# Abhipray/audio-codec

Measured on AMD Instinct MI355X. Metric: audio channel-frames/s encode (48 kHz, 1024-line long blocks, 128 kb/s/ch), higher is better.
Workload: dtype f64

## Files before the change

### audio-codec_amd/csrc/k_psy.hip

```cpp
#include "pacx_launch.h"
#include "mdct_dev.h"
#include "pcm_stage.h"
#include "wave_np_sum.h"
#include "quant_dev.h"


template <int DT>
__device__ __forceinline__ double hann_sample(const typename PcmStage<DT>::elem *raw, int i,
                                              const double *__restrict__ hw,
                                              const double *__restrict__ hw_pcm)
{
    if constexpr (DT == 0) {
        const int c = raw[i];
        return hw_pcm[i] * (double)(c == -32768 ? 0 : c);
    } else {
        return hw[i] * raw[i];
    }
}

#ifdef PACX_PSY_DEBUG
__device__ long long g_psy_dbg[16 * 16];
#define PSY_T(k) do { long long t_; asm volatile("s_waitcnt lgkmcnt(0)\n\ts_memtime %0\n\ts_waitcnt lgkmcnt(0)" : "=s"(t_) :: "memory"); \
                      if (dbg_on) dbg_acc[k] += t_ - dbg_last; dbg_last = t_; } while (0)
extern "C" int pacx_debug_read_psy(long long *out, int n)
// ... 4 lines not shown
                       if (lane == 0 && side_last) atomicAdd((unsigned long long *)&g_psy_dbg[128 + (k)], (unsigned long long)(t_ - side_last)); \
                       side_last = t_; } while (0)
#else
#define PSY_T(k) do { } while (0)
#define SIDE_T(k) do { } while (0)
#endif

#ifdef MASK_NOINLINE_RT
__device__ __attribute__((noinline)) double mask_round_trip(double x) { return pacx_spl_of_intensity_of(x); }
#else
__device__ __forceinline__ double mask_round_trip(double x) { return pacx_spl_of_intensity_of(x); }
#endif

__device__ __forceinline__ PacxPeak make_peak(double left, double centre, int f, double fstep)
{
    const double e = left + centre;
    const double spl = pacx_spl_scalar(e);
    const double avg = (((double)(f - 1) * fstep) * left + ((double)f * fstep) * centre) / e;
    PacxPeak p;
    p.z = pacx_bark(avg);
    p.spl = spl;
    p.slope = -27.0 + 0.367 * fmax(spl - 40.0, 0.0);
    return p;
}

template <int DT> struct SideLongLds {
    typedef typename PcmStage<DT>::elem E;
    static constexpr int RAW_BYTES = (int)sizeof(E) * PACX_N_LONG;
    static constexpr int A_BYTES = 1024;
    static constexpr int B_BYTES = RAW_BYTES > 1032 * 8 ? RAW_BYTES : 1032 * 8;
    static constexpr int BYTES = A_BYTES + B_BYTES;
};

__device__ __forceinline__ void fft512n_g2(cplx a[8], cplx b[8], cplx *tile, const cplx tw1[7], const cplx tw2[7],
                                           int lane)
{
    dft8(a);
    dft8(b);
#pragma unroll
    for (int k1 = 1; k1 < 8; ++k1) {
        const cplx w = tw1[k1 - 1];
        a[k1] = c_mul(a[k1], w);
        b[k1] = c_mul(b[k1], w);
    }
    fft512n_x1_write(tile, a, lane);
    wave_lds_fence();
    fft512n_x1_read(tile, a, lane);
    fft512n_x1_write(tile, b, lane);
    dft8(a);
    wave_lds_fence();
    fft512n_x1_read(tile, b, lane);
    dft8(b);
#pragma unroll
    for (int k2 = 1; k2 < 8; ++k2) {
        const cplx w = tw2[k2 - 1];
        a[k2] = c_mul(a[k2], w);
        b[k2] = c_mul(b[k2], w);
    }
    fft512n_x2_write(tile, a, lane);
    wave_lds_fence();
    fft512n_x2_read(tile, a, lane);
    fft512n_x2_write(tile, b, lane);
    dft8(a);
    wave_lds_fence();
    fft512n_x2_read(tile, b, lane);
    wave_lds_fence();
    dft8(b);
}

__device__ __forceinline__ double bperm_f64(double v, int src_lane)
{
    const int lo = __builtin_amdgcn_ds_bpermute(src_lane << 2, __double2loint(v));
    const int hi = __builtin_amdgcn_ds_bpermute(src_lane << 2, __double2hiint(v));
    return __hiloint2double(hi, lo);
}

__device__ __forceinline__ double pair_intensity(cplx a, cplx bz, cplx w, double norm)
{
    const cplx s = make_double2(a.x + bz.x, a.y - bz.y);
    const cplx d = make_double2(a.x - bz.x, a.y + bz.y);
    const cplx wd = c_mul(w, d);
    const double xr = 0.5 * (s.x + wd.y), xi = 0.5 * (s.y - wd.x);
    return norm * fma(xr, xr, xi * xi);
}

__device__ __forceinline__ void load_lane_twiddles(const PacxTables &T, int lane, cplx tw1[7], cplx tw2[7])
{
#pragma unroll
    for (int k = 1; k < 8; ++k) {
        tw1[k - 1] = T.w512[(lane * k) & 511];
        tw2[k - 1] = T.w512[(8 * (lane & 7) * k) & 511];
    }
}

struct FrontArgs {
    const short *src;
    double *lines;
    int32_t *scale_out;
    uint32_t *status;
};
struct MdctOperands {
    int q[16];
    double w[16];
    cplx twl[8];
};

__device__ __forceinline__ void mdct_fetch(const PacxTables &T, const short *__restrict__ src, int lane,
                                           MdctOperands &m)
{
    const double *__restrict__ win = T.win_long;
#pragma unroll
    for (int j = 0; j < 4; ++j) {
        const int4 t = *(const int4 *)(src + 8 * (lane + 64 * j));
        m.q[4 * j] = t.x; m.q[4 * j + 1] = t.y; m.q[4 * j + 2] = t.z; m.q[4 * j + 3] = t.w;
    }
#pragma unroll
    for (int n1 = 0; n1 < 8; ++n1) {
        int i0, i1, i2, i3, ia, ib;
        mdct_fold_index<PACX_N_LONG>(n1, lane + 64 * n1, i0, i1, i2, i3);
        mdct_fold_sym_index(n1, i0, i1, i2, i3, ia, ib);
        m.w[2 * n1] = win[ia];
        m.w[2 * n1 + 1] = win[ib];
    }
#pragma unroll
    for (int k = 0; k < 8; ++k)
        m.twl[k] = T.tw_long[lane + 64 * k];
}

__device__ __forceinline__ void mdct_long_one(const PacxTables &T, long long cf, char *regB, int lane,
                                              const MdctOperands &m, double *__restrict__ lines,
                                              int32_t *__restrict__ scale_out, uint32_t *__restrict__ status)
{
    short *raw = (short *)regB;
    cplx *tile = (cplx *)regB;
    cplx tw1[7], tw2[7];
#pragma unroll
    for (int k = 1; k < 8; ++k)
        tw1[k - 1] = T.w512[(lane * k) & 511];
#pragma unroll
    for (int j = 0; j < 4; ++j)
        *(int4 *)(raw + 8 * (lane + 64 * j)) = make_int4(m.q[4 * j], m.q[4 * j + 1], m.q[4 * j + 2], m.q[4 * j + 3]);
    wave_lds_fence();
    cplx v[8];
    for (int pass = 0;; ++pass) {
        int lowest = 0;
#pragma unroll
        for (int n1 = 0; n1 < 8; ++n1) {
            int i0, i1, i2, i3;
            mdct_fold_index<PACX_N_LONG>(n1, lane + 64 * n1, i0, i1, i2, i3);
            double c0, c1, c2, c3;
            mdct_fold_codes<false>(raw, i0, i1, i2, i3, c0, c1, c2, c3, lowest);
            const double wa = m.w[2 * n1] * MDCT_LONG_KSCALE, wb = m.w[2 * n1 + 1] * MDCT_LONG_KSCALE;
            v[n1] = c_mul(mdct_fold_sym(n1, wa, wb, c0, c1, c2, c3), m.twl[n1]);
        }
        if (pass || !__builtin_amdgcn_ballot_w64(lowest == -32768))
            break;
        wave_lds_fence();
        mdct_zero_min_codes((unsigned *)raw, lane);
        wave_lds_fence();
    }
#pragma unroll
    for (int k = 1; k < 8; ++k)
        tw2[k - 1] = T.w512[(8 * (lane & 7) * k) & 511];
    wave_lds_fence();
    fft512n(v, tile, tw1, 1, tw2, 1, lane);
    mdct_long_epilogue(T, v, [&](int k3) { return m.twl[k3]; }, cf, lane, lines, scale_out, PACX_SUB, status);
}

template <int DT, bool FAST, bool FRONT = false>
__device__ __forceinline__ void side_long_one(const PacxTables &T, const PacxPcmView &in, long long cf,
                                              char *regA, char *regB, int lane,
                                              PacxPeak *__restrict__ peaks, int32_t *__restrict__ n_peaks,
                                              int32_t *__restrict__ n_kept_out,
                                              double *__restrict__ sbr_mean,
                                              int32_t *__restrict__ sbr_overall,
                                              const FrontArgs *fa = nullptr)
{
    typedef typename PcmStage<DT>::elem E;
    cplx *tile = (cplx *)regB;
    double *inten = (double *)regB;
    E *raw = (E *)regB;

#ifdef PACX_PSY_DEBUG
    long long side_last = 0;
#endif
    SIDE_T(15);
    const double *__restrict__ hw = T.hann_long, *__restrict__ hwp = T.hann_long_pcm;
    cplx ev[8], od[8];
    cplx tw1[7], tw2[7];
    load_lane_twiddles(T, lane, tw1, tw2);
    if constexpr (DT == 0 && FAST) {
        const long long f = cf / in.n_ch;
        const int ch = (int)(cf - f * in.n_ch);
        const short *src = (const short *)in.base + f * in.frame_stride + ch * in.ch_stride;
        int2 q[8];
#pragma unroll
        for (int n1 = 0; n1 < 8; ++n1)
            q[n1] = *(const int2 *)(src + 4 * (lane + 64 * n1));
        SIDE_T(0);
#pragma unroll
        for (int n1 = 0; n1 < 8; ++n1) {
            const int i = 4 * (lane + 64 * n1);
            const double2 h01 = *(const double2 *)(hwp + i), h23 = *(const double2 *)(hwp + i + 2);
            const int c0 = (short)(q[n1].x & 0xFFFF), c1 = q[n1].x >> 16;
            const int c2 = (short)(q[n1].y & 0xFFFF), c3 = q[n1].y >> 16;
            ev[n1] = make_double2(h01.x * (double)(c0 == -32768 ? 0 : c0), h01.y * (double)(c1 == -32768 ? 0 : c1));
            od[n1] = make_double2(h23.x * (double)(c2 == -32768 ? 0 : c2), h23.y * (double)(c3 == -32768 ? 0 : c3));
        }
    } else {
        stage_samples<DT, FAST>(raw, in, cf, 0, PACX_N_LONG, lane);
        wave_lds_fence();
        SIDE_T(0);
#pragma unroll
        for (int n1 = 0; n1 < 8; ++n1) {
            const int i = 4 * (lane + 64 * n1);
            ev[n1] = make_double2(hann_sample<DT>(raw, i, hw, hwp), hann_sample<DT>(raw, i + 1, hw, hwp));
            od[n1] = make_double2(hann_sample<DT>(raw, i + 2, hw, hwp), hann_sample<DT>(raw, i + 3, hw, hwp));
        }
        wave_lds_fence();
    }
    SIDE_T(1);
    fft512n_g2(ev, od, tile, tw1, tw2, lane);
    SIDE_T(2);
    const int mirror = (64 - lane) & 63;
    constexpr int AHEAD = 2;
    cplx w1q[8], w2q[8];
#pragma unroll
    for (int k3 = 0; k3 < AHEAD; ++k3) {
        w1q[k3] = T.w1024[lane + 64 * k3];
        w2q[k3] = T.w2048[lane + 64 * k3];
    }
#pragma unroll
    for (int k3 = 0; k3 < 8; ++k3) {
        const int k = lane + 64 * k3;
        if (k3 + AHEAD < 8) {
            w1q[k3 + AHEAD] = T.w1024[k + 64 * AHEAD];
            w2q[k3 + AHEAD] = T.w2048[k + 64 * AHEAD];
        }
        const cplx w1k = w1q[k3], w2k = w2q[k3];
        const cplx t = c_mul(w1k, od[k3]);
        const cplx zk = c_add(ev[k3], t), zk5 = c_sub(ev[k3], t);
        cplx pe, po;
        pe.x = bperm_f64(ev[7 - k3].x, mirror);
        pe.y = bperm_f64(ev[7 - k3].y, mirror);
        po.x = bperm_f64(od[7 - k3].x, mirror);
        po.y = bperm_f64(od[7 - k3].y, mirror);
        if (lane == 0) {
            pe = ev[(8 - k3) & 7];
            po = od[(8 - k3) & 7];
        }
        const cplx tm = c_mul(make_double2(-w1k.x, w1k.y), po);
        cplx zm = c_add(pe, tm), zm5 = c_sub(pe, tm);
        if (k == 0) {
            zm5 = zk;
            zm = zk5;
// ... 148 lines not shown
            const double mean = wave_np_sum(inten + T.band_lower_long[b], cnt, lane) / (double)cnt;
            if (lane == 0)
                sbr_mean[cf * PACX_SUB + (b - first)] = mean;
        }
        if (lane == 0) {
            const int sf = pacx_scale_factor(sqrt(mx / T.norm_long) / (double)PACX_M_LONG, T.n_scale_bits, 5);
            if (sf < sbr_overall[cf * PACX_SUB])
                sbr_overall[cf * PACX_SUB] = sf;
        }
    }
}

template <int DT, bool FAST>
__global__ __launch_bounds__(64, DT == 0 ? 3 : 2) void k_side_long(PacxTables T, PacxPcmView in,
                                                 const uint8_t *__restrict__ flags, long long n_cf,
                                                 int skip_cur, PacxPeak *__restrict__ peaks,
                                                 int32_t *__restrict__ n_peaks,
                                                 int32_t *__restrict__ n_kept_out,
                                                 double *__restrict__ sbr_mean,
                                                 int32_t *__restrict__ sbr_overall)
{
    __shared__ __attribute__((aligned(16))) char regA[SideLongLds<DT>::A_BYTES];
    __shared__ __attribute__((aligned(16))) char regB[SideLongLds<DT>::B_BYTES];
    const long long cf = pacx_xcd_frame(blockIdx.x, gridDim.x, n_cf);
    if (cf >= n_cf)
        return;
    const unsigned fl = flags ? flags[cf / in.n_ch] : 0u;
    if (skip_cur && (fl & 2u))
        return;
    side_long_one<DT, FAST>(T, in, cf, regA, regB, threadIdx.x, peaks, n_peaks, n_kept_out, sbr_mean,
                            sbr_overall);
}

__global__ __launch_bounds__(64, 3) void k_front_long(PacxTables T, PacxPcmView in, long long n_cf,
                                                      double *__restrict__ lines, int32_t *__restrict__ scale_out,
                                                      uint32_t *__restrict__ status, PacxPeak *__restrict__ peaks,
                                                      int32_t *__restrict__ n_peaks, int32_t *__restrict__ n_kept_out)
{
    __shared__ __attribute__((aligned(16))) char regA[SideLongLds<0>::A_BYTES];
    __shared__ __attribute__((aligned(16))) char regB[SideLongLds<0>::B_BYTES];
    static_assert(SideLongLds<0>::B_BYTES >= (int)sizeof(cplx) * WFFT_TILE_N, "region B holds the FFT tile");
    const long long cf = pacx_xcd_frame(blockIdx.x, gridDim.x, n_cf);
    if (cf >= n_cf)
        return;
    const int lane = threadIdx.x;
    if (lane == 0)
        status[cf] = 0u;
    if (lane >= 1 && lane < PACX_SUB)
        scale_out[cf * PACX_SUB + lane] = 0;
    const long long f = cf / in.n_ch;
    const int ch = (int)(cf - f * in.n_ch);
    FrontArgs fa;
    fa.src = (const short *)in.base + f * in.frame_stride + ch * in.ch_stride;
    fa.lines = lines;
    fa.scale_out = scale_out;
    fa.status = status;
    side_long_one<0, true, true>(T, in, cf, regA, regB, lane, peaks, n_peaks, n_kept_out, nullptr, nullptr,
                                 &fa);
}

template <int DT, bool FAST>
__global__ __launch_bounds__(64) void k_side_short(PacxTables T, PacxPcmView in,
                                                  const uint8_t *__restrict__ flags, long long n_cf,
                                                  int only_cur, PacxPeak *__restrict__ peaks,
                                                  int32_t *__restrict__ n_peaks,
                                                  int32_t *__restrict__ n_kept_out)
{
// ... 710 lines not shown
```

### audio-codec_amd/_lib.py

```python
import ctypes
import os

HERE = os.path.dirname(os.path.abspath(__file__))
LIB_PATH = os.environ.get("PACX_LIB") or os.path.join(HERE, "libpacx.so")

PACX_ABI_VERSION = 7
PCM_I16, PCM_F64 = 0, 1
FLAG_LAST, FLAG_CUR, FLAG_NEXT = 1, 2, 4
ST_SHORT, ST_ZERO_SUBBLOCK, ST_ALLOC_CAP, ST_VQ_UNDEFINED, ST_GUARD, ST_MALFORMED = 1, 2, 4, 8, 16, 32
ST_REF_RAISES = 64
ST_RATE_CAP = 128
RATE_STEP = 32
RATE_TARGET_GRID = 64
BAND_CAND = 16
PROFILE_MAX = 8193
SEG_CF_MAX = 1 << 40
E_ARG, E_UNSUPPORTED = -1, -2
REF_SCALAR_SBR_ERROR = "'numpy.int64' object does not support item assignment"
MAX_BANDS = 32
SUB = 8

c_double_p = ctypes.POINTER(ctypes.c_double)
c_int32_p = ctypes.POINTER(ctypes.c_int32)

# ... 144 lines not shown
    "profile_segments": [_I64, _I64, _D, _D, _P, _P],
    "pick": [_D, _P, _P, _P, _P],
    "pick_segments": [_I64, _I64, _P, _P, _P, _P, _P],
    "thresholds": [_D, _D, _P, _P, _P, _P],
    "pick_thresholds": [_D, _D, _D, _P, _P, _P, _P],
    "pick_thresholds_segments": [_I64, _I64, _D, _D, _P, _P, _P, _P, _P],
}
SIGNATURES.update({f"pacx_{kind}_{op}": (ctypes.c_int, [_P, _I64, *head, _P, _P, _P, *tail])
                   for kind, head in CURVE_HEADS.items() for op, tail in CURVE_TAILS.items()})


class PacxBucket(ctypes.Structure):
    _fields_ = [("drain_q16", ctypes.c_int64), ("size_bytes", ctypes.c_int64), ("start_q16", ctypes.c_int64)]


BUCKET_Q = 16
BUCKET_SIZE_MAX = 1 << 40
BUCKET_RESULT = ("total", "peak_q16", "peak_hop", "first_over", "end_q16")
BUCKET_SIGNATURES = {"pacx_bucket_scan": (ctypes.c_int, [_P, _I64, ctypes.c_int32, _P, ctypes.POINTER(PacxBucket), _P, _P,
                                                         _P])}
BUCKET_SIGNATURES.update({f"pacx_{kind}_solve_bucket": (ctypes.c_int, [_P, _I64, ctypes.c_int32, *head, _P, _P, _P, _I64,
                                                                       ctypes.POINTER(PacxBucket), _D, _D, _P, _P, _P, _P,
                                                                       _P, _P])
                          for kind, head in CURVE_HEADS.items()})
PIN_PHASES_MAX = 16
PIN_RESULT = ("phases", "open")
BUCKET_PIN_SIGNATURES = {"pacx_bucket_through": (ctypes.c_int, [_P, _I64, ctypes.c_int32, _P, ctypes.POINTER(PacxBucket), _P,
                                                                _P, _P, _P])}
BUCKET_PIN_SIGNATURES.update({f"pacx_{kind}_solve_bucket_pinned": (ctypes.c_int, [_P, _I64, ctypes.c_int32, *head, _P, _P, _P,
                                                                                  _I64, ctypes.POINTER(PacxBucket), _D, _D,
                                                                                  ctypes.c_int32, ctypes.c_int32, _P, _P,
                                                                                  _P, _P, _P, _P, _P, _P, _P])
                              for kind, head in CURVE_HEADS.items()})
NMR_MAX_BANDS, NMR_COUNT, NMR_AUDIBLE, NMR_MAX, NMR_HIST, NMR_HIST_BINS = 32, 0, 1, 2, 3, 320
NMR_HIST_LO, NMR_HIST_STEP = -120.0, 0.5
NMR_SUMMARY_WORDS = NMR_HIST + NMR_HIST_BINS + 2
INDEX_SEGMENT = 8192
(WIN_SINE, WIN_START, WIN_STOP, WIN_STARTSTOP, WIN_SINE_SHORT, WIN_HANN, WIN_HANN_SHORT, WIN_KBD,
 WIN_KBD_SHORT) = range(9)
MDCT_SHORT, MDCT_PREWINDOWED, MDCT_KBD = 1, 2, 4

_lib = None


class PacxError(RuntimeError):
    pass


def load():
    global _lib
    if _lib is not None:
        return _lib
    from . import build as _build
    if os.environ.get("PACX_LIB"):
        if _build._read(LIB_PATH + ".hash") != _build.library_hash():
            raise PacxError(f"{LIB_PATH} (PACX_LIB) was not built from the sources in this tree: rebuild it with "
                            "`python audio-codec_amd/build.py --variant ...` / `--phase-debug`")
    elif not _build.is_current():
        if os.environ.get("PACX_AUTOBUILD") == "1":
            import sys
            print("audio_codec_amd: libpacx.so is missing or stale -- rebuilding (PACX_AUTOBUILD=1)", file=sys.stderr,
                  flush=True)
            try:
                _build.build(verbose=False)
            except Exception as e:
                raise PacxError(f"libpacx.so is missing or stale and could not be rebuilt: {e}") from e
        else:
            raise PacxError("libpacx.so is missing or does not belong to the sources in this tree (content hash "
                            "mismatch): run `python audio-codec_amd/build.py` (or set PACX_AUTOBUILD=1).  "
                            "There is no CPU implementation of this path.")
    if not os.path.exists(LIB_PATH):
        raise PacxError(
            f"{LIB_PATH} not found: build it with `python audio-codec_amd/build.py` "
            "(hipcc, gfx950).  There is no CPU implementation of this path.")
    import torch
    lib = ctypes.CDLL(LIB_PATH)
    for name, (res, args) in {**SIGNATURES, **BUCKET_SIGNATURES, **BUCKET_PIN_SIGNATURES}.items():
        fn = getattr(lib, name)
        fn.restype = res
        fn.argtypes = args
    if lib.pacx_abi_version() != PACX_ABI_VERSION:
        raise PacxError("libpacx.so ABI version does not match the Python binding")
    _lib = lib
    return lib


def check(lib, handle, rc, what):
    if rc != 0:
        msg = lib.pacx_last_error(handle)
        raise PacxError(f"{what} failed ({rc}): {msg.decode() if msg else '?'}")
```

### audio-codec_amd/build.py

```python
import fcntl
import hashlib
import json
import os
import re
import subprocess
import sys
from concurrent.futures import ThreadPoolExecutor

HERE = os.path.dirname(os.path.abspath(__file__))
CSRC = os.path.join(HERE, "csrc")
OUT = os.path.join(HERE, "libpacx.so")
OBJ = os.path.join(HERE, "build")
RESOURCES = os.path.join(OBJ, "resources.json")
SOURCES = ["pacx_api.hip", "k_mdct.hip", "k_psy.hip", "k_quant.hip", "k_misc.hip", "k_mdct2.hip", "k_decode.hip",
           "k_vq.hip", "k_vq_dec.hip", "k_mdct3.hip", "k_index.hip", "k_nmr.hip", "k_rate.hip", "k_band.hip",
           "k_vq_band.hip", "k_profile.hip", "k_seg_profile.hip", "k_rate_profile.hip", "k_kept.hip",
           "k_bucket.hip", "k_bucket_pin.hip"]
FLAGS = ["-O3", "-std=c++17", "--offload-arch=gfx950", "-fPIC", "-ffp-contract=off",
         "-Wall", "-Wno-unused-function", "-Rpass-analysis=kernel-resource-usage"]


def _hipcc():
    return os.environ.get("HIPCC", "/opt/rocm/bin/hipcc")


def _headers():
    hs = sorted(os.path.join(CSRC, f) for f in os.listdir(CSRC) if f.endswith(".h"))
    hs += [os.path.join(HERE, "..", "include", f) for f in ("pacx.h", "pacx_bucket.h", "pacx_bucket_pin.h")]
    return hs


def _digest(paths, extra=()):
    h = hashlib.sha256()
    for e in extra:
        h.update(e.encode() + b"\0")
    for p in paths:
        h.update(os.path.basename(p).encode() + b"\0")
        with open(p, "rb") as f:
            h.update(f.read())
    return h.hexdigest()


def _read(path):
    try:
        with open(path) as f:
            return f.read().strip()
    except OSError:
        return None


def source_hashes(extra_flags=()):
    hs = _headers()
    return {s: _digest([os.path.join(CSRC, s)] + hs, FLAGS + list(extra_flags)) for s in SOURCES}


def library_hash():
    sh = source_hashes()
    return hashlib.sha256("".join(sh[s] for s in SOURCES).encode()).hexdigest()


def is_current():
# ... 189 lines not shown
```

### audio-codec_amd/csrc/k_misc.hip

```cpp
#include "pacx_launch.h"

__global__ void k_window(const double *__restrict__ win, long long n_rows, int len,
                         const double *__restrict__ x, double *__restrict__ y)
{
    const long long i = (long long)blockIdx.x * blockDim.x + threadIdx.x;
    if (i < n_rows * len)
        y[i] = win[i % len] * x[i];
}

__global__ void k_quant_elem(int op, long long n, const double *__restrict__ x, int scale, int a, int b,
                             int64_t *__restrict__ out)
{
    const long long i = (long long)blockIdx.x * blockDim.x + threadIdx.x;
    if (i >= n)
        return;
    const double v = x[i];
    if (op == 0) {
        const int64_t mag = pacx_quant_mag(fabs(v), a);
        out[i] = (v < 0.0 ? ((int64_t)1 << (a - 1)) : 0) + mag;
    } else if (op == 1) {
        out[i] = pacx_scale_factor(fabs(v), a, b);
    } else if (op == 2) {
        out[i] = pacx_mantissa(v, scale, a, b);
    } else {
        out[i] = pacx_mantissa_fp(v, scale, a, b);
    }
}

__global__ void k_dequant_elem(int op, long long n, const int64_t *__restrict__ codes, int scale, int a, int b,
                               double *__restrict__ out)
{
    const long long i = (long long)blockIdx.x * blockDim.x + threadIdx.x;
    if (i >= n)
// ... 290 lines not shown
    if (lane == 63) {
        ws[wv] = ss;
        wl[wv] = sl;
    }
    __syncthreads();
    int at_s = ss - ns, at_l = sl - nl, all_s = 0, all_l = 0;
#pragma unroll
    for (int w = 0; w < NW; ++w) {
        at_s += w < wv ? ws[w] : 0;
        at_l += w < wv ? wl[w] : 0;
        all_s += ws[w];
        all_l += wl[w];
    }
    for (int j = 0; j < per; ++j) {
        if (!((valid >> j) & 1ull))
            break;
        const long long f = f0 + j;
        if ((shorts >> j) & 1ull) {
            for (int c = 0; c < n_ch; ++c)
                list_short[at_s * n_ch + c] = (int32_t)(f * n_ch + c);
            ++at_s;
        } else {
            for (int c = 0; c < n_ch; ++c)
                list_long[at_l * n_ch + c] = (int32_t)(f * n_ch + c);
            ++at_l;
        }
    }
    if (tid == 0) {
        counts[0] = all_l * n_ch;
        counts[1] = all_s * n_ch;
    }
}

void pacx_k::pacx_launch_frame_lists(const uint8_t *flags, long long n_frames, int n_ch, int32_t *list_long,
                             int32_t *list_short, int32_t *counts, hipStream_t st)
{
    if (n_frames <= 0)
        return;
    if (n_frames <= LISTS_SMALL_MAX) {
        hipLaunchKernelGGL(k_frame_lists_small, dim3(1), dim3(LISTS_SMALL_THREADS), 0, st, flags, n_frames, n_ch, list_long,
                           list_short, counts);
        return;
    }
    (void)hipMemsetAsync(counts, 0, 2 * sizeof(int32_t), st);
    hipLaunchKernelGGL(k_frame_lists, dim3((unsigned)((n_frames + 255) / 256)), dim3(256), 0, st, flags, n_frames,
                       n_ch, list_long, list_short, counts);
}

void pacx_k::pacx_launch_transient_f64(long long n_blocks, int n_ch, int n, const double *blocks, double thresh, uint8_t *out,
                               hipStream_t st)
{
    if (n_blocks > 0)
        hipLaunchKernelGGL(k_transient_f64, dim3((unsigned)n_blocks), dim3(64), 0, st, n_blocks, n_ch, n, blocks, thresh,
                           out);
}

void pacx_k::pacx_launch_transient(const PacxPcmView &in, long long n_hops, int hop, uint8_t *transient,
                           uint8_t *flags, hipStream_t st)
{
    if (n_hops > 0)
        hipLaunchKernelGGL(k_transient, dim3((unsigned)n_hops), dim3(64), 0, st, in, n_hops, hop, transient);
    if (flags)
        hipLaunchKernelGGL(k_stream_flags, dim3((unsigned)((n_hops + 2 + 255) / 256)), dim3(256), 0, st,
                           transient, n_hops, flags);
}

// ... 40 lines not shown
```

### audio-codec_amd/csrc/pacx_api.hip

```cpp
#include <hip/hip_runtime.h>

#include <math.h>
#include <stdio.h>
#include <stdlib.h>
#include <string.h>

#include <cmath>
#include <string>
#include <vector>

#include "../../include/pacx.h"
#include "body_index.h"
#include "pacx_launch.h"
#include "pvq_dev.h"
#include "pacx_vq_tables.h"
#include "pacx_tables_gen.h"

using namespace pacx_k;

struct PacxOverrides {
    int split_short;
    int fuse_tail;
    int fuse_front;
    int vq_fuse_alloc;
    int vq_frame;
    int vq_bfs;
    int vq_dec_frame;
};

#define PACX_FUSE_FRONT_DEFAULT 1

static int env_override(const char *name, int lo, int hi)
{
    const char *e = getenv(name);
    if (!e || !*e)
        return -1;
    char *end;
    const long v = strtol(e, &end, 10);
    return (*end || v < lo || v > hi) ? -1 : (int)v;
}

static PacxOverrides read_overrides(void)
{
    PacxOverrides o;
    o.split_short = env_override("PACX_SPLIT_SHORT", 0, 0);
// ... 229 lines not shown
    int n_dev = 0;
    if (hipGetDeviceCount(&n_dev) != hipSuccess || n_dev <= 0)
        return fail(nullptr, PACX_E_HIP, "pacx_create: no HIP device visible (this library has no CPU path)");
    if (cfg->device < 0 || cfg->device >= n_dev)
        return fail(nullptr, PACX_E_ARG, "pacx_create: device ordinal out of range");

    pacx_handle *h = new pacx_handle();
    h->device = cfg->device;
    h->force = read_overrides();
    h->tables_exact = 1;
    memset(&h->T, 0, sizeof(h->T));
    int rc = PACX_OK;
#define TRY(x) do { rc = (x); if (rc) { g_create_err = h->err; pacx_destroy(h); return rc; } } while (0)
    {
        hipError_t e = hipSetDevice(cfg->device);
        if (e != hipSuccess) {
            g_create_err = std::string("hipSetDevice: ") + hipGetErrorString(e);
            delete h;
            return PACX_E_HIP;
        }
    }
    if (hipStreamCreateWithFlags(&h->side_stream, hipStreamNonBlocking) != hipSuccess ||
        hipEventCreateWithFlags(&h->ev_fork, hipEventDisableTiming) != hipSuccess ||
        hipEventCreateWithFlags(&h->ev_join, hipEventDisableTiming) != hipSuccess ||
        hipStreamCreateWithFlags(&h->short_stream, hipStreamNonBlocking) != hipSuccess ||
        hipStreamCreateWithFlags(&h->spare_stream, hipStreamNonBlocking) != hipSuccess ||
        hipEventCreateWithFlags(&h->ev_short_done, hipEventDisableTiming) != hipSuccess ||
        hipEventCreateWithFlags(&h->ev_lists, hipEventDisableTiming) != hipSuccess) {
        g_create_err = "pacx_create: could not create the side stream / events";
        pacx_destroy(h);
        return PACX_E_HIP;
    }
    {
        hipDeviceProp_t prop;
        h->n_cu = (hipGetDeviceProperties(&prop, cfg->device) == hipSuccess && prop.multiProcessorCount > 0)
                      ? prop.multiProcessorCount : 256;
    }
    PacxTables &T = h->T;
    const int NL = PACX_N_LONG, NS = PACX_N_SHORT, ML = PACX_M_LONG, MS = PACX_M_SHORT;
    const double sr = cfg->sample_rate;

    std::vector<double> wl(4 * NL), ws(NS), hl(NL), hs(NS);
    if (cfg->win_long) {
        memcpy(wl.data(), cfg->win_long, sizeof(double) * 4 * NL);
    } else {
        const std::vector<double> sl = gen_table(PACX_GEN_SINE_LONG, NL), ss = gen_table(PACX_GEN_SINE_SHORT, NS);
        const int pad = NL / 4 - NS / 4;
        for (int i = 0; i < NL; ++i) {
            wl[i] = sl[i];
            double st;
            if (i < NL / 2) st = sl[i];
            else if (i < NL / 2 + pad) st = 1.0;
            else if (i < NL / 2 + pad + NS / 2) st = ss[NS / 2 + (i - NL / 2 - pad)];
            else st = 0.0;
            wl[NL + i] = st;
            double ssw;
            if (i < pad) ssw = 0.0;
            else if (i < pad + NS / 2) ssw = ss[i - pad];
            else if (i < pad + NS / 2 + 2 * pad) ssw = 1.0;
            else if (i < pad + NS + 2 * pad) ssw = ss[NS / 2 + (i - pad - NS / 2 - 2 * pad)];
            else ssw = 0.0;
            wl[3 * NL + i] = ssw;
        }
        for (int i = 0; i < NL; ++i)
            wl[2 * NL + i] = wl[NL + (NL - 1 - i)];
    }
// ... 757 lines not shown
        return post_launch_forked(h, what);
    }
    if (!mixed && fast && (h->force.fuse_front >= 0 ? h->force.fuse_front : PACX_FUSE_FRONT_DEFAULT)) {
        s.front_long(st);
        s.mask(0, fuse ? &mt : nullptr, st);
        if (!fuse)
            tail(s.list_short, s.counts + 1, fuse, st);
        return post_launch(h, what);
    }
    const bool one_stream = !h->fork_side;
    hipStream_t side_st = one_stream ? st : h->side_stream;
    if (!one_stream) {
        HIP_TRY_FORKED(h, hipEventRecord(h->ev_fork, st));
        HIP_TRY_FORKED(h, hipStreamWaitEvent(h->side_stream, h->ev_fork, 0));
    }
    s.side(0, false, side_st);
    if (!one_stream)
        HIP_TRY_FORKED(h, hipEventRecord(h->ev_join, h->side_stream));
    s.mdct(st);
    if (!one_stream)
        HIP_TRY_FORKED(h, hipStreamWaitEvent(st, h->ev_join, 0));
    s.mask(0, fuse ? &mt : nullptr, st);
    if (!fuse || mixed)
        tail(s.list_short, s.counts + 1, fuse, st);
    return post_launch_forked(h, what);
}

extern "C" int pacx_set_side_fork(pacx_handle *h, int enable)
{
    if (!h)
        return PACX_E_ARG;
    h->fork_side = enable ? 1 : 0;
    return PACX_OK;
}

extern "C" int pacx_encode_batch(pacx_handle *h, const pacx_pcm *in, const uint8_t *frame_flags,
                                 int32_t *overall_scale, int32_t *scale_factor, int32_t *bit_alloc,
                                 int32_t *mantissa, uint32_t *status, void *stream)
{
    return encode_scalar(h, in, frame_flags, overall_scale, scale_factor, bit_alloc, mantissa, status, nullptr,
                         nullptr, stream, "pacx_encode_batch");
}

extern "C" int pacx_encode_pack_batch(pacx_handle *h, const pacx_pcm *in, const uint8_t *frame_flags,
                                      int32_t *overall_scale, int32_t *scale_factor, int32_t *bit_alloc,
                                      int32_t *mantissa, uint32_t *status, uint8_t *payload, int32_t *n_bytes,
                                      void *stream)
{
    if (h && in && in->n_frames > 0 && (!payload || !n_bytes))
        return fail(h, PACX_E_ARG, "pacx_encode_pack_batch: payload and n_bytes are required");
    return encode_scalar(h, in, frame_flags, overall_scale, scale_factor, bit_alloc, mantissa, status, payload,
                         n_bytes, stream, "pacx_encode_pack_batch");
}

extern "C" int pacx_encode_vq_batch(pacx_handle *h, const pacx_pcm *in, const uint8_t *frame_flags,
                                    int32_t *overall_scale, int32_t *bit_alloc, uint8_t *payload,
                                    int32_t *n_bytes, uint32_t *status, pacx_vq_entry *entries,
                                    int32_t *entry_count, int32_t entries_per_band, void *stream)
{
    if (!h)
        return PACX_E_ARG;
    EncodeStep s(h, frame_flags, stream);
    int rc = s.view(in);
    if (rc || s.n_cf == 0)
        return rc;
    if (!overall_scale || !bit_alloc || !payload || !n_bytes || !status)
// ... 1492 lines not shown
```

### audio-codec_amd/csrc/pacx_launch.h

```cpp
#ifndef PACX_LAUNCH_H
#define PACX_LAUNCH_H

#include "../../include/pacx.h"
#include "pacx_dev.h"

struct PvqTables;

namespace pacx_k {

void pacx_launch_mdct(const PacxTables &T, const PacxPcmView &in, int dtype, int fast,
                      const uint8_t *flags, long long n_cf, int short_blocks, int mixed, int prewin,
                      double *lines, int32_t *scale_out, int scale_stride, uint32_t *status,
                      hipStream_t st);
void pacx_launch_mdct_v2(const PacxTables &T, const PacxPcmView &in, const uint8_t *flags, long long n_cf,
                         int skip_cur, double *lines, int32_t *scale_out, int scale_stride,
                         uint32_t *status_init, int n_cu, const int32_t *cf_list, const int32_t *cf_count,
                         hipStream_t st);
void pacx_launch_mdct_x2(const PacxTables &T, const PacxPcmView &in, long long n_cf, double *lines,
                         int32_t *scale_out, int scale_stride, uint32_t *status_init, int n_cu, hipStream_t st);

void pacx_launch_side(const PacxTables &T, const PacxPcmView &in, int dtype, int fast,
                      const uint8_t *flags, long long n_cf, int short_blocks, int mixed,
                      PacxPeak *peaks, int32_t *n_peaks, int32_t *n_kept, double *sbr_mean,
                      int32_t *sbr_overall, hipStream_t st);
// ... 17 lines not shown
                          uint32_t *status, hipStream_t st);
void pacx_launch_quantize(const PacxTables &T, const uint8_t *flags, int n_ch, long long n_cf,
                          int short_blocks, int mixed, const double *lines, const int32_t *overall,
                          int overall_stride, const int32_t *bit_alloc, int32_t *scale_factor,
                          int32_t *mantissa, hipStream_t st);
void pacx_launch_pack(const PacxTables &T, const uint8_t *flags, int n_ch, long long n_cf,
                      const int32_t *overall, const int32_t *scale_factor, const int32_t *bit_alloc,
                      const int32_t *mantissa, const uint32_t *status, uint8_t *payload,
                      int payload_stride, int32_t *n_bytes, hipStream_t st);
void pacx_launch_tail(const PacxTables &T, const uint8_t *flags, int n_ch, long long n_cf, const double *smr,
                      const double *lines, const int32_t *overall, int32_t *bit_alloc, int32_t *scale_factor,
                      int32_t *mantissa, uint32_t *status, uint8_t *payload, int payload_stride,
                      int32_t *n_bytes, const int32_t *list_short, const int32_t *count_short, int skip_long,
                      hipStream_t st);
void pacx_launch_gather(long long n_cf, const uint8_t *payload, int payload_stride,
                        const int32_t *n_bytes, long long *chunk_buf, long long *offs_buf, uint8_t *body,
                        long long capacity, long long *total, hipStream_t st);

void pacx_launch_frame_lists(const uint8_t *flags, long long n_frames, int n_ch, int32_t *list_long,
                             int32_t *list_short, int32_t *counts, hipStream_t st);
void pacx_launch_window(const double *win, long long n_rows, int len, const double *x, double *y,
                        hipStream_t st);
void pacx_launch_quant_elem(int op, long long n, const double *x, int scale, int a, int b, int64_t *out,
                            hipStream_t st);
void pacx_launch_dequant_elem(int op, long long n, const int64_t *codes, int scale, int a, int b, double *out,
                              hipStream_t st);
void pacx_launch_mdct_direct(long long n_rows, int a, int b, int inverse, const double *x, double *y, hipStream_t st);
void pacx_launch_bitalloc_generic(long long n, int nb, const int32_t *n_lines, const double *budget,
                                  int max_mant, const double *smr, int32_t *bits, hipStream_t st);
void pacx_launch_transient_f64(long long n_blocks, int n_ch, int n, const double *blocks, double thresh, uint8_t *out,
                               hipStream_t st);
void pacx_launch_transient(const PacxPcmView &in, long long n_hops, int hop, uint8_t *transient,
                           uint8_t *flags, hipStream_t st);

void pacx_launch_imdct_plain(const PacxTables &T, long long n_rows, int short_blocks, const double *lines,
                             double *blocks, hipStream_t st);
void pacx_launch_sbr_scalar_lines(const PacxTables &T, long long n_cf, const uint8_t *cf_flags,
                                  const int32_t *scale_factor, const int32_t *bit_alloc, const int32_t *mantissa,
                                  double *lines, uint8_t *sbr_flag, int routing, hipStream_t st);
void pacx_launch_unpack(const PacxTables &T, long long n_cf, const uint8_t *payload, int payload_stride,
                        const long long *offsets, const int32_t *n_bytes, uint8_t *flags_out, int32_t *overall,
                        int32_t *scale_factor, int32_t *bit_alloc, int32_t *mantissa, uint32_t *status,
                        hipStream_t st);
void pacx_launch_decode(const PacxTables &T, long long n_blocks, int n_ch, const uint8_t *cf_flags,
                        const int32_t *overall, const int32_t *scale_factor, const int32_t *bit_alloc,
                        const int32_t *mantissa, const double *lines_in, double *blocks, int16_t *pcm,
                        hipStream_t st);
void pacx_launch_ola_tail(long long n_blocks, int n_ch, const double *blocks, double *tail, int flush, int16_t *pcm,
                          hipStream_t st);

size_t pacx_index_ws_bytes(long long n_body, PacxIndexWs *ws);
void pacx_launch_index(const PacxIndexWs &ws, char *mem, const uint8_t *body, long long n_body, int n_ch, int final,
                       long long max_records, long long *offsets, int32_t *n_bytes, long long *result, hipStream_t st);

void pacx_launch_nmr(const PacxTables &T, const uint8_t *flags, int n_ch, long long n_cf, const double *lines,
                     const double *dec_lines, const int32_t *overall, const double *thr, const uint32_t *status,
                     double *noise, double *mask, double *nmr_db, hipStream_t st);
void pacx_launch_nmr_summary(const PacxTables &T, const uint8_t *flags, int n_ch, long long n_cf,
                             const double *nmr_db, unsigned long long *summary, hipStream_t st);

void pacx_launch_rate_search(const PacxTables &T, const uint8_t *flags, int n_ch, long long n_cf,
                             double target_nmr_db, double max_bits_per_sample, const double *lines,
                             const double *thr, const double *smr, const int32_t *overall, int32_t *budget,
                             int32_t *bit_alloc, uint32_t *status, hipStream_t st);
void pacx_launch_bitalloc_budget(const PacxTables &T, const uint8_t *flags, int n_ch, long long n_cf,
                                 const int32_t *budget, const double *smr, int32_t *bit_alloc, uint32_t *status,
// ... 233 lines not shown
```

### audio-codec_amd/engine.py

```python
import ctypes
import os

import numpy as np
import torch

from . import _lib, tables
from .curves import BAND, RATE
from .psychoac import ScaleFactorBands, AssignMDCTLinesFromFreqLimits

N_LONG, N_SHORT = 1024, 128


def _ptr(t):
    return ctypes.c_void_p(t.data_ptr()) if t is not None else None


class PcmView:

    def __init__(self, tensor, n_channels, n_frames, frame_stride, channel_stride,
                 sample_stride=1):
        if tensor.dtype == torch.int16:
            dt = _lib.PCM_I16
        elif tensor.dtype == torch.float64:
            dt = _lib.PCM_F64
# ... 992 lines not shown
        n_out = a + b if inverse else (a + b) // 2
        x = x.contiguous().view(-1, n_in)
        out = self._empty((x.shape[0], n_out), torch.float64)
        self._call("pacx_mdct_direct_batch", ctypes.c_int64(x.shape[0]), int(a), int(b), int(bool(inverse)), _ptr(x),
                   _ptr(out), self._stream())
        return out

    def transient_detect(self, blocks, thresh=4.5):
        blocks = blocks.contiguous()
        n, n_ch, ln = blocks.shape
        out = self._empty((n,), torch.uint8)
        self._call("pacx_transient_detect_f64", ctypes.c_int64(n), int(n_ch), int(ln), _ptr(blocks),
                   ctypes.c_double(float(thresh)), _ptr(out), self._stream())
        return out

    def bit_alloc_generic(self, budget, max_mant_bits, n_lines, smr):
        smr = smr.contiguous()
        n, nb = smr.shape
        nl = torch.as_tensor(np.asarray(n_lines, dtype=np.int32), device=self.device)
        bits = self._empty((n, nb), torch.int32)
        self._call("pacx_bitalloc_generic", ctypes.c_int64(n), int(nb), _ptr(nl), _ptr(budget.contiguous()),
                   int(max_mant_bits), _ptr(smr), _ptr(bits), self._stream())
        return bits


class EncoderPool:

    def __init__(self, n, *args, **kwargs):
        self.encs = [Encoder(*args, **kwargs) for _ in range(max(1, int(n)))]
        dev = self.encs[0].device
        self.streams = [torch.cuda.Stream(device=dev) for _ in self.encs]
        self.done = [torch.cuda.Event() for _ in self.encs]
        self._turn = 0
        self._gate = self._gate_stream = None
        self._used = [False] * len(self.encs)
        if len(self.encs) > 1:
            for e in self.encs:
                e.set_side_fork(True)

    def __len__(self):
        return len(self.encs)

    def next(self):
        k = self._turn
        self._turn = (k + 1) % len(self.encs)
        return k

    def slot(self, k):
        pool = self

        class _Slot:
            def __enter__(self_inner):
                self_inner.ctx = torch.cuda.stream(pool.streams[k])
                self_inner.ctx.__enter__()
                return pool.encs[k]

            def __exit__(self_inner, *exc):
                pool.done[k].record(pool.streams[k])
                pool._used[k] = True
                return self_inner.ctx.__exit__(*exc)
        return _Slot()

    def align(self, delay_us=None):
        if len(self.encs) < 2:
            return
        if delay_us is None:
            delay_us = float(os.environ.get("PACX_POOL_GATE_US", "100"))
        if delay_us <= 0 or not hasattr(torch.cuda, "_sleep"):
            return
        dev = self.encs[0].device
        if self._gate is None:
            self._gate_stream = torch.cuda.Stream(device=dev)
            self._gate = torch.cuda.Event()
            t0, t1 = torch.cuda.Event(enable_timing=True), torch.cuda.Event(enable_timing=True)
            with torch.cuda.stream(self._gate_stream):
                torch.cuda._sleep(100_000)
                t0.record()
                torch.cuda._sleep(2_000_000)
                t1.record()
            t1.synchronize()
            self._cycles_per_us = 2_000_000 / max(t0.elapsed_time(t1) * 1e3, 1.0)
        with torch.cuda.stream(self._gate_stream):
            for k in range(len(self.encs)):
                if self._used[k]:
                    self._gate_stream.wait_event(self.done[k])
            torch.cuda._sleep(int(delay_us * self._cycles_per_us))
            self._gate.record(self._gate_stream)
        for s in self.streams:
            s.wait_event(self._gate)

    def wait(self, k, stream=None):
        (stream or torch.cuda.current_stream(self.encs[0].device)).wait_event(self.done[k])

    def synchronize(self):
        for s in self.streams:
            s.synchronize()

    def close(self):
        for e in self.encs:
            e.close()
```

### include/pacx.h

```cpp
#ifndef PACX_H
#define PACX_H

#include <stdint.h>

#ifdef __cplusplus
extern "C" {
#endif

#define PACX_ABI_VERSION 7

#define PACX_OK            0
#define PACX_E_ARG        -1
#define PACX_E_UNSUPPORTED -2
#define PACX_E_HIP        -3
#define PACX_E_NOMEM      -4

#define PACX_PCM_I16 0
#define PACX_PCM_F64 1

#define PACX_FLAG_LAST 1u
#define PACX_FLAG_CUR  2u
#define PACX_FLAG_NEXT 4u

#define PACX_WIN_SINE 0
// ... 339 lines not shown
                             const int64_t *limit_bytes, double nmr_lo_db, double nmr_hi_db, int32_t *budget,
                             int32_t *n_bytes, uint8_t *capped, pacx_rate_result *result, void *stream);
int pacx_band_solve_segments(pacx_handle *h, int64_t n_cf, const double *nmr, const int32_t *cap,
                             const int32_t *cap_alloc, int64_t n_seg, const int64_t *seg_first,
                             const int64_t *limit_bytes, double nmr_lo_db, double nmr_hi_db, int32_t *bit_alloc,
                             int32_t *n_bytes, uint8_t *capped, pacx_rate_result *result, void *stream);


int pacx_rate_solve_peak(pacx_handle *h, int64_t n_cf, int32_t row, int32_t sub_stride, const double *worst,
                         const int32_t *bits, const int32_t *steps, int64_t n_seg, const int64_t *seg_first,
                         const int64_t *peak_bytes, int64_t limit_bytes, double nmr_lo_db, double nmr_hi_db,
                         int32_t *budget, int32_t *n_bytes, uint8_t *capped, int32_t *floor, pacx_rate_result *result,
                         pacx_rate_result *result_stream, void *stream);
int pacx_band_solve_peak(pacx_handle *h, int64_t n_cf, const double *nmr, const int32_t *cap, const int32_t *cap_alloc,
                         int64_t n_seg, const int64_t *seg_first, const int64_t *peak_bytes, int64_t limit_bytes,
                         double nmr_lo_db, double nmr_hi_db, int32_t *bit_alloc, int32_t *n_bytes, uint8_t *capped,
                         int32_t *floor, pacx_rate_result *result, pacx_rate_result *result_stream, void *stream);

int pacx_encode_pack_alloc_batch(pacx_handle *h, const pacx_pcm *in, const uint8_t *frame_flags,
                                 const int32_t *bit_alloc_in, int32_t *overall_scale, int32_t *scale_factor,
                                 int32_t *bit_alloc, int32_t *mantissa, uint32_t *status, uint8_t *payload,
                                 int32_t *n_bytes, void *stream);


int pacx_vq_band_curve_batch(pacx_handle *h, const pacx_pcm *in, const uint8_t *frame_flags, double max_bits_per_sample,
                             double *nmr, int32_t *cap, int32_t *cap_alloc, void *stream);

int pacx_encode_vq_alloc_batch(pacx_handle *h, const pacx_pcm *in, const uint8_t *frame_flags,
                               const int32_t *bit_alloc_in, int32_t *overall_scale, int32_t *bit_alloc,
                               uint8_t *payload, int32_t *n_bytes, uint32_t *status, void *stream);

#include "pacx_bucket.h"
#include "pacx_bucket_pin.h"

#ifdef __cplusplus
}
#endif
#endif
```

Before: 53.04 million.

## Defer twiddle loads to cut register pressure and raise front_long occupancy

Moves the MDCT long twiddle loads out of the prefetched operand struct into the compute routine. The second-stage FFT twiddles are now loaded just before they are needed, reusing one register array for both stages. In the fused front kernel, tw2 is fetched inside the first FFT stage, and an asm barrier pins the FFT results in registers. Launch bounds go from 3 to 4 waves per SIMD. The aim is to shorten live ranges so the kernel fits more waves, at the cost of less latency hiding for the deferred loads and possible spills under the tighter register budget.

```diff
diff --git a/audio-codec_amd/csrc/k_psy.hip b/audio-codec_amd/csrc/k_psy.hip
--- a/audio-codec_amd/csrc/k_psy.hip
+++ b/audio-codec_amd/csrc/k_psy.hip
@@ -60,8 +60,9 @@
     static constexpr int BYTES = A_BYTES + B_BYTES;
 };
 
+template <class F>
 __device__ __forceinline__ void fft512n_g2(cplx a[8], cplx b[8], cplx *tile, const cplx tw1[7], const cplx tw2[7],
-                                           int lane)
+                                           F fetch_tw2, int lane)
 {
     dft8(a);
     dft8(b);
@@ -71,6 +72,7 @@
         a[k1] = c_mul(a[k1], w);
         b[k1] = c_mul(b[k1], w);
     }
+    fetch_tw2();
     fft512n_x1_write(tile, a, lane);
     wave_lds_fence();
     fft512n_x1_read(tile, a, lane);
@@ -112,13 +114,17 @@
     return norm * fma(xr, xr, xi * xi);
 }
 
-__device__ __forceinline__ void load_lane_twiddles(const PacxTables &T, int lane, cplx tw1[7], cplx tw2[7])
-{
-#pragma unroll
-    for (int k = 1; k < 8; ++k) {
+__device__ __forceinline__ void load_lane_tw1(const PacxTables &T, int lane, cplx tw1[7])
+{
+#pragma unroll
+    for (int k = 1; k < 8; ++k)
         tw1[k - 1] = T.w512[(lane * k) & 511];
+}
+__device__ __forceinline__ void load_lane_tw2(const PacxTables &T, int lane, cplx tw2[7])
+{
+#pragma unroll
+    for (int k = 1; k < 8; ++k)
         tw2[k - 1] = T.w512[(8 * (lane & 7) * k) & 511];
-    }
 }
 
 struct FrontArgs {
@@ -130,7 +136,6 @@
 struct MdctOperands {
     int q[16];
     double w[16];
-    cplx twl[8];
 };
 
 __device__ __forceinline__ void mdct_fetch(const PacxTables &T, const short *__restrict__ src, int lane,
@@ -150,9 +155,6 @@
         m.w[2 * n1] = win[ia];
         m.w[2 * n1 + 1] = win[ib];
     }
-#pragma unroll
-    for (int k = 0; k < 8; ++k)
-        m.twl[k] = T.tw_long[lane + 64 * k];
 }
 
 __device__ __forceinline__ void mdct_long_one(const PacxTables &T, long long cf, char *regB, int lane,
@@ -161,13 +163,13 @@
 {
     short *raw = (short *)regB;
     cplx *tile = (cplx *)regB;
-    cplx tw1[7], tw2[7];
-#pragma unroll
-    for (int k = 1; k < 8; ++k)
-        tw1[k - 1] = T.w512[(lane * k) & 511];
 #pragma unroll
     for (int j = 0; j < 4; ++j)
         *(int4 *)(raw + 8 * (lane + 64 * j)) = make_int4(m.q[4 * j], m.q[4 * j + 1], m.q[4 * j + 2], m.q[4 * j + 3]);
+    cplx twl[8];
+#pragma unroll
+    for (int k = 0; k < 8; ++k)
+        twl[k] = T.tw_long[lane + 64 * k];
     wave_lds_fence();
     cplx v[8];
     for (int pass = 0;; ++pass) {
@@ -179,7 +181,7 @@
             double c0, c1, c2, c3;
             mdct_fold_codes<false>(raw, i0, i1, i2, i3, c0, c1, c2, c3, lowest);
             const double wa = m.w[2 * n1] * MDCT_LONG_KSCALE, wb = m.w[2 * n1 + 1] * MDCT_LONG_KSCALE;
-            v[n1] = c_mul(mdct_fold_sym(n1, wa, wb, c0, c1, c2, c3), m.twl[n1]);
+            v[n1] = c_mul(mdct_fold_sym(n1, wa, wb, c0, c1, c2, c3), twl[n1]);
         }
         if (pass || !__builtin_amdgcn_ballot_w64(lowest == -32768))
             break;
@@ -187,12 +189,24 @@
         mdct_zero_min_codes((unsigned *)raw, lane);
         wave_lds_fence();
     }
-#pragma unroll
-    for (int k = 1; k < 8; ++k)
-        tw2[k - 1] = T.w512[(8 * (lane & 7) * k) & 511];
-    wave_lds_fence();
-    fft512n(v, tile, tw1, 1, tw2, 1, lane);
-    mdct_long_epilogue(T, v, [&](int k3) { return m.twl[k3]; }, cf, lane, lines, scale_out, PACX_SUB, status);
+    cplx tw[7];
+    load_lane_tw1(T, lane, tw);
+    wave_lds_fence();
+    dft8(v);
+    fft512n_twiddle(v, tw, 1);
+    load_lane_tw2(T, lane, tw);
+    fft512n_x1_write(tile, v, lane);
+    wave_lds_fence();
+    fft512n_x1_read(tile, v, lane);
+    wave_lds_fence();
+    dft8(v);
+    fft512n_twiddle(v, tw, 1);
+    fft512n_x2_write(tile, v, lane);
+    wave_lds_fence();
+    fft512n_x2_read(tile, v, lane);
+    wave_lds_fence();
+    dft8(v);
+    mdct_long_epilogue(T, v, [&](int k3) { return twl[k3]; }, cf, lane, lines, scale_out, PACX_SUB, status);
 }
 
 template <int DT, bool FAST, bool FRONT = false>
@@ -216,7 +230,9 @@
     const double *__restrict__ hw = T.hann_long, *__restrict__ hwp = T.hann_long_pcm;
     cplx ev[8], od[8];
     cplx tw1[7], tw2[7];
-    load_lane_twiddles(T, lane, tw1, tw2);
+    load_lane_tw1(T, lane, tw1);
+    if constexpr (!FRONT)
+        load_lane_tw2(T, lane, tw2);
     if constexpr (DT == 0 && FAST) {
         const long long f = cf / in.n_ch;
         const int ch = (int)(cf - f * in.n_ch);
@@ -248,7 +264,15 @@
         wave_lds_fence();
     }
     SIDE_T(1);
-    fft512n_g2(ev, od, tile, tw1, tw2, lane);
+    fft512n_g2(ev, od, tile, tw1, tw2, [&] {
+        if constexpr (FRONT)
+            load_lane_tw2(T, lane, tw2);
+    }, lane);
+    if constexpr (FRONT) {
+#pragma unroll
+        for (int k = 0; k < 8; ++k)
+            asm volatile("" : "+v"(ev[k].x), "+v"(ev[k].y), "+v"(od[k].x), "+v"(od[k].y));
+    }
     SIDE_T(2);
     const int mirror = (64 - lane) & 63;
     constexpr int AHEAD = 2;
@@ -463,7 +487,7 @@
                             sbr_overall);
 }
 
-__global__ __launch_bounds__(64, 3) void k_front_long(PacxTables T, PacxPcmView in, long long n_cf,
+__global__ __launch_bounds__(64, 4) void k_front_long(PacxTables T, PacxPcmView in, long long n_cf,
                                                       double *__restrict__ lines, int32_t *__restrict__ scale_out,
                                                       uint32_t *__restrict__ status, PacxPeak *__restrict__ peaks,
                                                       int32_t *__restrict__ n_peaks, int32_t *__restrict__ n_kept_out)
```

After: 55.48 million, median of 6. 1.05x the previous value.

## Replace pool gate stream sleep with per-stream wall-clock hold kernel

Applied to the files above, without the earlier changes.

The pool's align step used to route every stream through a separate gate stream that slept for a calibrated cycle count and then released all encoder streams through one event. It now has each stream wait on the other streams' done events and launch its own small hold kernel. These kernels agree on a shared wall-clock deadline through a CAS on a generation-tagged word and spin until it passes. This drops the cross-stream event hop and the cycle calibration, so the streams should be released together at a common deadline. In exchange it adds a spinning single-wave kernel per stream and atomic coordination logic that depends on all streams reaching the hold within the slack window.

```diff
diff --git a/audio-codec_amd/_lib.py b/audio-codec_amd/_lib.py
--- a/audio-codec_amd/_lib.py
+++ b/audio-codec_amd/_lib.py
@@ -200,6 +200,8 @@
                                                                                   ctypes.c_int32, ctypes.c_int32, _P, _P,
                                                                                   _P, _P, _P, _P, _P, _P, _P])
                               for kind, head in CURVE_HEADS.items()})
+HOLD_MAX_US, HOLD_TICKS_PER_US = 1.0e6, 100
+HOLD_SIGNATURES = {"pacx_hold": (ctypes.c_int, [_P, _P, ctypes.c_int32, _D, _P, _P])}
 NMR_MAX_BANDS, NMR_COUNT, NMR_AUDIBLE, NMR_MAX, NMR_HIST, NMR_HIST_BINS = 32, 0, 1, 2, 3, 320
 NMR_HIST_LO, NMR_HIST_STEP = -120.0, 0.5
 NMR_SUMMARY_WORDS = NMR_HIST + NMR_HIST_BINS + 2
@@ -243,7 +245,7 @@
             "(hipcc, gfx950).  There is no CPU implementation of this path.")
     import torch
     lib = ctypes.CDLL(LIB_PATH)
-    for name, (res, args) in {**SIGNATURES, **BUCKET_SIGNATURES, **BUCKET_PIN_SIGNATURES}.items():
+    for name, (res, args) in {**SIGNATURES, **BUCKET_SIGNATURES, **BUCKET_PIN_SIGNATURES, **HOLD_SIGNATURES}.items():
         fn = getattr(lib, name)
         fn.restype = res
         fn.argtypes = args
diff --git a/audio-codec_amd/build.py b/audio-codec_amd/build.py
--- a/audio-codec_amd/build.py
+++ b/audio-codec_amd/build.py
@@ -26,7 +26,7 @@
 
 def _headers():
     hs = sorted(os.path.join(CSRC, f) for f in os.listdir(CSRC) if f.endswith(".h"))
-    hs += [os.path.join(HERE, "..", "include", f) for f in ("pacx.h", "pacx_bucket.h", "pacx_bucket_pin.h")]
+    hs += [os.path.join(HERE, "..", "include", f) for f in ("pacx.h", "pacx_bucket.h", "pacx_bucket_pin.h", "pacx_hold.h")]
     return hs
 
 
diff --git a/audio-codec_amd/csrc/hold_word.h b/audio-codec_amd/csrc/hold_word.h
--- /dev/null
+++ b/audio-codec_amd/csrc/hold_word.h
@@ -0,0 +1,45 @@
+#ifndef PACX_HOLD_WORD_H
+#define PACX_HOLD_WORD_H
+
+#include <stdint.h>
+
+#if defined(__HIPCC__)
+#define HOLD_HD __host__ __device__ __forceinline__
+#else
+#define HOLD_HD static inline
+#endif
+
+#define HOLD_TICK_BITS 48
+#define HOLD_TICK_MASK ((UINT64_C(1) << HOLD_TICK_BITS) - 1)
+#define HOLD_TICKS_PER_US 100
+#define HOLD_MAX_US 1.0e6
+#define HOLD_SLACK_TICKS 1024
+
+HOLD_HD uint64_t hold_word(unsigned gen, uint64_t deadline)
+{
+    return ((uint64_t)(gen & 0xFFFFu) << HOLD_TICK_BITS) | (deadline & HOLD_TICK_MASK);
+}
+
+HOLD_HD unsigned hold_word_gen(uint64_t word) { return (unsigned)(word >> HOLD_TICK_BITS); }
+
+HOLD_HD uint64_t hold_word_deadline(uint64_t word) { return word & HOLD_TICK_MASK; }
+
+HOLD_HD unsigned hold_next_gen(unsigned gen) { return (gen + 1u) & 0xFFFFu; }
+
+HOLD_HD int64_t hold_tick_diff(uint64_t a, uint64_t b)
+{
+    const uint64_t d = (a - b) & HOLD_TICK_MASK;
+    return (d >> (HOLD_TICK_BITS - 1)) ? (int64_t)d - ((int64_t)1 << HOLD_TICK_BITS) : (int64_t)d;
+}
+
+HOLD_HD uint64_t hold_adopt(uint64_t word, unsigned gen, uint64_t now, int64_t ticks, int *mine)
+{
+    *mine = hold_word_gen(word) == (gen & 0xFFFFu);
+    const uint64_t own = (now + (uint64_t)ticks) & HOLD_TICK_MASK;
+    if (!*mine)
+        return own;
+    const uint64_t d = hold_word_deadline(word);
+    return hold_tick_diff(d, own) > HOLD_SLACK_TICKS ? own : d;
+}
+
+#endif
diff --git a/audio-codec_amd/csrc/k_misc.hip b/audio-codec_amd/csrc/k_misc.hip
--- a/audio-codec_amd/csrc/k_misc.hip
+++ b/audio-codec_amd/csrc/k_misc.hip
@@ -1,4 +1,5 @@
 #include "pacx_launch.h"
+#include "hold_word.h"
 
 __global__ void k_window(const double *__restrict__ win, long long n_rows, int len,
                          const double *__restrict__ x, double *__restrict__ y)
@@ -355,6 +356,48 @@
     }
 }
 
+#define HOLD_MAX_TRIES 64
+__global__ __launch_bounds__(64) void k_hold(unsigned long long *word, unsigned gen, long long ticks, long long *debug)
+{
+    if (threadIdx.x != 0)
+        return;
+    uint64_t now = (uint64_t)wall_clock64() & HOLD_TICK_MASK;
+    int mine = 0;
+    uint64_t deadline = 0;
+    unsigned long long seen = __hip_atomic_load(word, __ATOMIC_RELAXED, __HIP_MEMORY_SCOPE_AGENT);
+    for (int tries = 0; tries < HOLD_MAX_TRIES; ++tries) {
+        deadline = hold_adopt(seen, gen, now, ticks, &mine);
+        if (mine)
+            break;
+        if (__hip_atomic_compare_exchange_strong(word, &seen, (unsigned long long)hold_word(gen, deadline), __ATOMIC_RELAXED,
+                                                 __ATOMIC_RELAXED, __HIP_MEMORY_SCOPE_AGENT))
+            break;
+    }
+    for (;;) {
+        const int64_t late = hold_tick_diff(now, deadline);
+        if (late >= 0 || late < -(int64_t)(ticks + HOLD_SLACK_TICKS))
+            break;
+        __builtin_amdgcn_s_sleep(2);
+        now = (uint64_t)wall_clock64() & HOLD_TICK_MASK;
+    }
+    if (debug) {
+        debug[0] = (long long)deadline;
+        debug[1] = (long long)now;
+    }
+}
+
+void pacx_k::pacx_launch_hold(void *word, unsigned gen, long long ticks, int64_t *debug, hipStream_t st)
+{
+    hipLaunchKernelGGL(k_hold, dim3(1), dim3(64), 0, st, (unsigned long long *)word, gen & 0xFFFFu, ticks,
+                       (long long *)debug);
+}
+
+hipError_t pacx_k::pacx_prepare_hold(void)
+{
+    hipFuncAttributes attr;
+    return hipFuncGetAttributes(&attr, reinterpret_cast<const void *>(k_hold));
+}
+
 void pacx_k::pacx_launch_frame_lists(const uint8_t *flags, long long n_frames, int n_ch, int32_t *list_long,
                              int32_t *list_short, int32_t *counts, hipStream_t st)
 {
diff --git a/audio-codec_amd/csrc/pacx_api.hip b/audio-codec_amd/csrc/pacx_api.hip
--- a/audio-codec_amd/csrc/pacx_api.hip
+++ b/audio-codec_amd/csrc/pacx_api.hip
@@ -11,6 +11,7 @@
 
 #include "../../include/pacx.h"
 #include "body_index.h"
+#include "hold_word.h"
 #include "pacx_launch.h"
 #include "pvq_dev.h"
 #include "pacx_vq_tables.h"
@@ -306,6 +307,14 @@
         return PACX_E_HIP;
     }
     {
+        hipError_t e = pacx_prepare_hold();
+        if (e != hipSuccess) {
+            g_create_err = std::string("pacx_create: the gate kernel could not be loaded: ") + hipGetErrorString(e);
+            pacx_destroy(h);
+            return PACX_E_HIP;
+        }
+    }
+    {
         hipDeviceProp_t prop;
         h->n_cu = (hipGetDeviceProperties(&prop, cfg->device) == hipSuccess && prop.multiProcessorCount > 0)
                       ? prop.multiProcessorCount : 256;
@@ -1129,6 +1138,19 @@
         return PACX_E_ARG;
     h->fork_side = enable ? 1 : 0;
     return PACX_OK;
+}
+
+extern "C" int pacx_hold(pacx_handle *h, void *word, int32_t gen, double delay_us, int64_t *debug, void *stream)
+{
+    if (!h)
+        return PACX_E_ARG;
+    if (!word || ((uintptr_t)word % 8) != 0 || ((uintptr_t)debug % 8) != 0)
+        return fail(h, PACX_E_ARG, "pacx_hold: word is null, or word or debug is not 8-byte aligned");
+    if (!(delay_us >= 0.0 && delay_us <= HOLD_MAX_US))
+        return fail(h, PACX_E_ARG, "pacx_hold: delay_us must lie in [0, 1e6]");
+    HIP_TRY(h, hipSetDevice(h->device));
+    pacx_launch_hold(word, (unsigned)gen & 0xFFFFu, llround(delay_us * HOLD_TICKS_PER_US), debug, (hipStream_t)stream);
+    return post_launch(h, "pacx_hold");
 }
 
 extern "C" int pacx_encode_batch(pacx_handle *h, const pacx_pcm *in, const uint8_t *frame_flags,
diff --git a/audio-codec_amd/csrc/pacx_launch.h b/audio-codec_amd/csrc/pacx_launch.h
--- a/audio-codec_amd/csrc/pacx_launch.h
+++ b/audio-codec_amd/csrc/pacx_launch.h
@@ -73,6 +73,8 @@
                                hipStream_t st);
 void pacx_launch_transient(const PacxPcmView &in, long long n_hops, int hop, uint8_t *transient,
                            uint8_t *flags, hipStream_t st);
+void pacx_launch_hold(void *word, unsigned gen, long long ticks, int64_t *debug, hipStream_t st);
+hipError_t pacx_prepare_hold(void);
 
 void pacx_launch_imdct_plain(const PacxTables &T, long long n_rows, int short_blocks, const double *lines,
                              double *blocks, hipStream_t st);
diff --git a/audio-codec_amd/engine.py b/audio-codec_amd/engine.py
--- a/audio-codec_amd/engine.py
+++ b/audio-codec_amd/engine.py
@@ -1048,7 +1048,10 @@
         self.streams = [torch.cuda.Stream(device=dev) for _ in self.encs]
         self.done = [torch.cuda.Event() for _ in self.encs]
         self._turn = 0
-        self._gate = self._gate_stream = None
+        self._gate = None
+        self._gate_word = torch.zeros(1, dtype=torch.int64).to(dev)
+        self._gate_gen = 0
+        self._gate_debug = None
         self._used = [False] * len(self.encs)
         if len(self.encs) > 1:
             for e in self.encs:
@@ -1082,28 +1085,21 @@
             return
         if delay_us is None:
             delay_us = float(os.environ.get("PACX_POOL_GATE_US", "100"))
-        if delay_us <= 0 or not hasattr(torch.cuda, "_sleep"):
+        if delay_us <= 0:
             return
-        dev = self.encs[0].device
+        for k in range(len(self.encs)):
+            if self._used[k]:
+                for j, s in enumerate(self.streams):
+                    if j != k:
+                        s.wait_event(self.done[k])
+        self._gate_gen = (self._gate_gen + 1) & 0xFFFF
+        for k, enc in enumerate(self.encs):
+            enc._call("pacx_hold", _ptr(self._gate_word), self._gate_gen, ctypes.c_double(float(delay_us)),
+                      _ptr(self._gate_debug[k]) if self._gate_debug is not None else None,
+                      ctypes.c_void_p(self.streams[k].cuda_stream))
         if self._gate is None:
-            self._gate_stream = torch.cuda.Stream(device=dev)
             self._gate = torch.cuda.Event()
-            t0, t1 = torch.cuda.Event(enable_timing=True), torch.cuda.Event(enable_timing=True)
-            with torch.cuda.stream(self._gate_stream):
-                torch.cuda._sleep(100_000)
-                t0.record()
-                torch.cuda._sleep(2_000_000)
-                t1.record()
-            t1.synchronize()
-            self._cycles_per_us = 2_000_000 / max(t0.elapsed_time(t1) * 1e3, 1.0)
-        with torch.cuda.stream(self._gate_stream):
-            for k in range(len(self.encs)):
-                if self._used[k]:
-                    self._gate_stream.wait_event(self.done[k])
-            torch.cuda._sleep(int(delay_us * self._cycles_per_us))
-            self._gate.record(self._gate_stream)
-        for s in self.streams:
-            s.wait_event(self._gate)
+        self._gate.record(self.streams[0])
 
     def wait(self, k, stream=None):
         (stream or torch.cuda.current_stream(self.encs[0].device)).wait_event(self.done[k])
diff --git a/include/pacx.h b/include/pacx.h
--- a/include/pacx.h
+++ b/include/pacx.h
@@ -395,6 +395,7 @@
 
 #include "pacx_bucket.h"
 #include "pacx_bucket_pin.h"
+#include "pacx_hold.h"
 
 #ifdef __cplusplus
 }
diff --git a/include/pacx_hold.h b/include/pacx_hold.h
--- /dev/null
+++ b/include/pacx_hold.h
@@ -0,0 +1,9 @@
+#ifndef PACX_HOLD_H
+#define PACX_HOLD_H
+#ifndef PACX_H
+#error "include pacx.h, which includes this header"
+#endif
+
+int pacx_hold(pacx_handle *h, void *word, int32_t gen, double delay_us, int64_t *debug, void *stream);
+
+#endif
```

New measurement: 52.84 million before, 53.61 million after, median of 6. +1.5%, better.
